# UniBwTAS/continuous_clustering

Measured on AMD Instinct MI355X. Metric: Mpoints/s clustered (64-beam streams), higher is better.
Workload: dtype f32

## Files before the change

continuous_clustering_amd/csrc/cc_device.h:

```cpp
#pragma once
#include <stdint.h>
#include <hip/hip_runtime.h>

#include "../../include/cc_hip.h"

namespace ccd
{

constexpr int WAVE = 64;
constexpr int MAX_ROWS_PER_LANE = 2;
constexpr int LINK_SLOTS = 4;
constexpr int WIN_COLS = 32;
constexpr int PP_SKIP = 0x7fffffff;
#ifndef CC_INS_WIN
#define CC_INS_WIN 64
#endif
constexpr int INS_WIN = CC_INS_WIN;
constexpr int SG_NAN = 1, SG_FOG = 2, SG_EGO = 4, SG_INCL_IGNORE = 8, SG_TOO_CLOSE = 16, SG_PENDING = 32;
constexpr unsigned NAN_RANGE_BITS = 0x7fc00001u;
#ifndef CC_TREE_SLOTS
#define CC_TREE_SLOTS 256
#endif
constexpr int TREE_SLOTS = CC_TREE_SLOTS;
#ifndef CC_TABLE_WAVES
// ... 47 lines not shown
    uint64_t exceed_one_rotation;
    uint64_t serial_columns;
    uint64_t stamp_alias_rounds;
    uint64_t batch_columns;
    uint64_t batch_bails;
    uint64_t batch_bail_reason[8];
    int64_t par_clear_done;
    int32_t par_bad;
    int32_t par_upto;
    int64_t serial_until;
    uint64_t dbg[16];
    int32_t error;
    int32_t n_events;
    int64_t error_a;
    int64_t error_b;
    int32_t n_links;
    int32_t pad2;
    int64_t overrun_col;
};

struct Planes
{
    float* dist;
    float* incl;
    float* incaz;
    uint16_t* gtag;
    uint32_t* src;
    uint8_t* inten;
    int32_t* trig;
    int64_t* colg;
    double* colminaz;
    uint8_t* ground;
    uint8_t* debug;
    uint8_t* ignored;
    int32_t* root;
    uint32_t* id;
    double* t_fin;
    uint32_t* t_width;
    uint32_t* t_pts;
    int32_t* t_uf;
    uint32_t* t_cid;
    int32_t* t_pos;
    uint8_t* t_finished;
    int32_t* ulist;
    int32_t* ucomp;
    unsigned long long* agg_fin;
    long long* agg_min;
// ... 65 lines not shown
```

continuous_clustering_amd/csrc/cc_engine.hip:

```cpp
#include <hip/hip_runtime.h>

#include <algorithm>
#include <chrono>
#include <cstdlib>
#include <cmath>
#include <cstdio>
#include <cstring>
#include <functional>
#include <limits>
#include <mutex>
#include <string>
#include <vector>

#include "cc_kernels.h"

#ifndef CC_LWAVE_MAX_STREAMS
#define CC_LWAVE_MAX_STREAMS 256
#endif

using namespace ccd;

struct cc_engine
{
    int device{0};
// ... 277 lines not shown
    e->d_small_seq = nullptr;
    e->d_input_sum = nullptr;
    e->small_view_ok = false;
    e->small_seq_expected = 0;
    free_pinned(e, PIN_SHAPE);
    return CC_OK;
}

int allocate(cc_engine* e)
{
    const Geometry& g = e->g;
    const size_t S = (size_t) g.num_streams;
    const size_t C = S * (size_t) g.cells;
    const size_t L = S * (size_t) g.ring_cols;
    const size_t T = S * (size_t) g.tree_capacity;
    Planes& P = e->P;
    int rc = CC_OK;
    e->slab_planning = getenv("CC_NO_SLAB") == nullptr;
    e->slab_bytes = 0;
    e->slab_plan.clear();
#define A(field, count)                                \
    if ((rc = alloc_plane(e, &P.field, (count))) != 0) \
        return rc;
    A(dist, C) A(incl, C) A(incaz, C) A(gtag, C) A(src, C) A(inten, C);
    A(trig, L) A(colg, L) A(colminaz, L);
    A(ground, C) A(debug, C) A(ignored, C) A(root, C) A(id, C);
    A(t_fin, C) A(t_width, C) A(t_pts, C) A(t_uf, C) A(t_cid, C) A(t_pos, C) A(t_finished, C);
    A(ulist, T) A(ucomp, T) A(agg_fin, T) A(agg_min, T) A(agg_max, T) A(agg_pts, T) A(agg_cid, T) A(agg_first, T) A(agg_flag, T);
    A(events, S * (size_t) g.event_capacity);
    A(sc_parent, C) A(sc_nlinks, C) A(sc_links, C) A(sc_fin, C);
    A(sc_term, C) A(col_newfin, L) A(col_info, L) A(col_act, L) A(pk_meta, C) A(pk_fin, C) A(pk_lk, C);
    A(sg_x2, C) A(sg_uz, C) A(sg_w, C) A(sg_flags, C) A(sc_rec, C);
    A(curtab, S * (size_t) g.num_rows);
    A(tab_acc, S * (size_t) g.tab_tiles * (size_t) g.num_rows);
    A(par_off, S * (size_t) cck::IP_MAXF);
    A(tabc, (size_t) BATCH_SLOTS * S * (size_t) g.tab_tiles * (size_t) g.num_rows);
    A(sc_visits, C);
    A(link_log, S * (size_t) g.link_capacity);
    A(sl_ctl, S * 4) A(sl_cols, L);
    if ((rc = alloc_plane(e, (unsigned long long**) &P.sl_rec, S * (size_t) cck::SL_CAP * sizeof(cck::ScanLongRec) / sizeof(unsigned long long))) != 0)
        return rc;
#undef A
    if ((rc = alloc_plane(e, &e->d_states, S)) != 0)
        return rc;
    if ((rc = alloc_plane(e, &e->d_par_left, 16)) != 0)
        return rc;
    if ((rc = alloc_plane(e, &e->d_bail_count, 4)) != 0)
// ... 31 lines not shown
    st.clear_done = -1;
    st.first_unpublished = -1;
    st.cluster_counter = 1;
    st.min_required = 0;
    st.finish_lower_bound = std::numeric_limits<double>::max();
    st.last_round_min_az = -1.0;
    st.overrun_col = std::numeric_limits<int64_t>::max();
    st.n_links = 0;
    for (auto& d : st.batch)
        d.seg_begin = d.seg_end = d.acp_next = d.pub_begin = d.pub_end = -1, d.mode = 0, d.fused = 0;
    st.assoc_mode = e->cfg.max_steps_in_row > WIN_COLS - 2 ? 1 : 0;
}

int reset_state(cc_engine* e, bool keep_table)
{
    e->small_view_ok = false;
    e->widest_steps_in_row = e->cfg.max_steps_in_row;
    std::fill(e->state_cached.begin(), e->state_cached.end(), 0);
    const Geometry& g = e->g;
    const size_t S = (size_t) g.num_streams;
    const size_t C = S * (size_t) g.cells;
    Planes& P = e->P;
    CC_HIP_CHECK(e, hipMemsetAsync(P.dist, 0xFF, C * sizeof(float), e->stream));
    CC_HIP_CHECK(e, hipMemsetAsync(P.incl, 0xFF, C * sizeof(float), e->stream));
    CC_HIP_CHECK(e, hipMemsetAsync(P.gtag, 0, C * sizeof(uint16_t), e->stream));
    CC_HIP_CHECK(e, hipMemsetAsync(P.id, 0, C * sizeof(uint32_t), e->stream));
    CC_HIP_CHECK(e, hipMemsetAsync(P.ground, CC_GP_UNKNOWN, C, e->stream));
    CC_HIP_CHECK(e, hipMemsetAsync(P.debug, CC_DBG_WHITE, C, e->stream));
    CC_HIP_CHECK(e, hipMemsetAsync(P.ignored, 0, C, e->stream));
    CC_HIP_CHECK(e, hipMemsetAsync(P.root, 0xFF, C * sizeof(int32_t), e->stream));
    CC_HIP_CHECK(e, hipMemsetAsync(P.tab_acc, 0, S * (size_t) g.tab_tiles * (size_t) g.num_rows * sizeof(unsigned long long), e->stream));
    CC_HIP_CHECK(e, hipMemsetAsync(P.sl_ctl, 0, S * 4 * sizeof(int32_t), e->stream));
    if (!keep_table)
        CC_HIP_CHECK(e, hipMemsetAsync(P.curtab, 0xFF, S * (size_t) g.num_rows * sizeof(float), e->stream));
    std::vector<StreamState> init(S);
    for (auto& st : init)
        fresh_stream_state(e, &st);
    CC_HIP_CHECK(e, hipMemcpyAsync(e->d_states, init.data(), S * sizeof(StreamState), hipMemcpyHostToDevice, e->stream));
    if (e->d_take_cursor)
        CC_HIP_CHECK(e, hipMemsetAsync(e->d_take_cursor, 0, 2 * S * sizeof(long long), e->stream));
    if (e->d_tc_cursor)
        CC_HIP_CHECK(e, hipMemsetAsync(e->d_tc_cursor, 0, 2 * S * sizeof(long long), e->stream));
    CC_HIP_CHECK(e, hipStreamSynchronize(e->stream));
    for (auto& v : e->pending_events)
        v.clear();
    for (auto& v : e->pending_links)
        v.clear();
    e->batch_open = false;
    for (bool& b : e->assoc_pending)
        b = false;
    e->deferred_tail = nullptr;
    e->lazy_pending = false;
    e->lazy_prev_left = nullptr;
    e->lazy_miss = 0;
    e->lazy_clean = 0;
    e->lazy_ok = true;
    return CC_OK;
}

int reset_streams_state(cc_engine* e, const std::vector<int>& list)
{
    const Geometry& g = e->g;
    const Planes& P = e->P;
    const unsigned long long cells = (unsigned long long) g.cells;
    cck::ResetJob job;
    memset(&job, 0, sizeof(job));
    const cck::ResetFill fills[cck::RESET_PLANES] = {
        {(char*) P.dist, cells * sizeof(float), 0xFF, 0},
        {(char*) P.incl, cells * sizeof(float), 0xFF, 0},
        {(char*) P.gtag, cells * sizeof(uint16_t), 0, 0},
        {(char*) P.id, cells * sizeof(uint32_t), 0, 0},
        {(char*) P.ground, cells, CC_GP_UNKNOWN, 0},
        {(char*) P.debug, cells, CC_DBG_WHITE, 0},
        {(char*) P.ignored, cells, 0, 0},
        {(char*) P.root, cells * sizeof(int32_t), 0xFF, 0},
        {(char*) P.tab_acc, (unsigned long long) g.tab_tiles * (unsigned long long) g.num_rows * sizeof(unsigned long long), 0, 0},
        {(char*) P.sl_ctl, 4 * sizeof(int32_t), 0, 0},
    };
    unsigned long long longest = 0;
    for (int k = 0; k < cck::RESET_PLANES; k++)
    {
        job.fill[k] = fills[k];
        longest = std::max(longest, fills[k].bytes);
    }
    fresh_stream_state(e, &job.fresh);
    job.states = e->d_states;
    job.take_cursor = e->d_take_cursor;
    job.tc_cursor = e->d_tc_cursor;
    job.num_streams = g.num_streams;
    int rc = ensure_gather(e, list.size() * sizeof(int));
    if (rc)
        return rc;
// ... 527 lines not shown
    const int64_t RC = e->g.ring_cols;
    const size_t off = (size_t) stream * (size_t) e->g.cells + (size_t) (st.overrun_col % RC) * R;
    if (hipMemcpy(col.data(), e->P.gtag + off, (size_t) R * sizeof(uint16_t), hipMemcpyDeviceToHost) != hipSuccess)
        return;
    const unsigned tag = 0x8000u | ((unsigned) (st.overrun_col / RC) & 0x7fffu);
    for (int row = R - 1; row >= 0; row--)
        if (col[(size_t) row] != tag && col[(size_t) row] != 0)
        {
            st.error_a = st.overrun_col - (int64_t) ((tag - (unsigned) col[(size_t) row]) & 0x7fffu) * RC;
            st.error_b = st.overrun_col;
            return;
        }
}

void restore_table_after_overrun(cc_engine* e, int stream, const StreamState& st)
{
    if (st.error != CC_ERR_RING_OVERRUN || st.overrun_col == std::numeric_limits<int64_t>::max())
        return;
    const int R = e->g.num_rows;
    const int64_t RC = e->g.ring_cols, c = st.overrun_col;
    const int64_t oldest = std::max<int64_t>(0, c - (RC - 2 * (int64_t) e->g.num_columns));
    const size_t base = (size_t) stream * (size_t) e->g.cells;
    float* curtab = e->P.curtab + (size_t) stream * (size_t) R;
    std::vector<float> table((size_t) R), incl, dist;
    std::vector<uint16_t> tags;
    std::vector<uint8_t> found((size_t) R, 0);
    if (hipMemcpy(table.data(), curtab, (size_t) R * sizeof(float), hipMemcpyDeviceToHost) != hipSuccess)
        return;
    int missing = R;
    for (int64_t hi = c - 1; hi >= oldest && missing > 0;)
    {
        const int64_t lo = std::max(std::max(oldest, hi - 255), hi - hi % RC);
        const size_t n = (size_t) (hi - lo + 1) * (size_t) R, off = base + (size_t) (lo % RC) * (size_t) R;
        incl.resize(n), dist.resize(n), tags.resize(n);
        if (hipMemcpy(incl.data(), e->P.incl + off, n * sizeof(float), hipMemcpyDeviceToHost) != hipSuccess ||
            hipMemcpy(dist.data(), e->P.dist + off, n * sizeof(float), hipMemcpyDeviceToHost) != hipSuccess ||
            hipMemcpy(tags.data(), e->P.gtag + off, n * sizeof(uint16_t), hipMemcpyDeviceToHost) != hipSuccess)
            return;
        for (int64_t g = hi; g >= lo && missing > 0; g--)
        {
            const unsigned tag = 0x8000u | ((unsigned) (g / RC) & 0x7fffu);
            const size_t o = (size_t) (g - lo) * (size_t) R;
            float below = 0.f;
            for (int row = R - 1; row >= 0; row--)
            {
                const bool has = tags[o + (size_t) row] == tag && !std::isnan(dist[o + (size_t) row]);
                const float cur = has ? incl[o + (size_t) row] : std::nanf("");
                const float diff = cur - below;
                if (!std::isnan(diff) && !found[(size_t) row])
                {
                    table[(size_t) row] = diff;
                    found[(size_t) row] = 1;
                    missing--;
                }
                below = cur;
            }
        }
        hi = lo - 1;
    }
    (void) hipMemcpy(curtab, table.data(), (size_t) R * sizeof(float), hipMemcpyHostToDevice);
}

void set_kernel_error(cc_engine* e, int stream, StreamState& st)
{
    fixup_overrun(e, stream, st);
    restore_table_after_overrun(e, stream, st);
    char buf[320];
    if (st.error == CC_ERR_RING_OVERRUN)
        snprintf(buf, sizeof(buf), "stream %d: This column is not cleared (ring buffer full or written after clearing): %lld, %lld, %d", stream,
                 (long long) st.error_a, (long long) st.error_b, e->g.ring_cols);
// ... 1711 lines not shown
```

continuous_clustering_amd/csrc/cc_k_base.h:

```cpp
#pragma once

#define CC_PI_F 3.14159274101257324219f
#define CC_2PI_D 6.283185307179586

__device__ __forceinline__ int lane_id()
{
    return threadIdx.x & 63;
}

__device__ __forceinline__ int f2i_x86(float v)
{
    if (!(v > -2147483904.0f && v < 2147483648.0f))
        return (int) 0x80000000;
    return (int) v;
}

template<int CTRL, int ROW_MASK>
__device__ __forceinline__ int dpp_mov_i32(int fill, int v)
{
    return __builtin_amdgcn_update_dpp(fill, v, CTRL, ROW_MASK, 0xf, false);
}
template<int CTRL, int ROW_MASK>
__device__ __forceinline__ long long dpp_mov_i64(long long fill, long long v)
{
// ... 210 lines not shown
    }
    return m;
}
__device__ __forceinline__ void caz_key(const float packed, int& kpos, int& kneg)
{
    const unsigned u = __float_as_uint(packed);
    const int k = (int) (u & 0x7fffffffu);
    if (u >> 31)
        kneg = k < kneg ? k : kneg;
    else
        kpos = k < kpos ? k : kpos;
}

constexpr uint16_t CELL_CLEARED = 0;
__device__ __forceinline__ uint16_t cell_tag(const long long pass)
{
    return (uint16_t) (0x8000u | ((unsigned) pass & 0x7fffu));
}

constexpr int IP_MAXF = 4608;

struct SP
{
    float *dist, *incl, *tabc;
    float* incaz;
    uint16_t* gtag;
    uint32_t* src;
    uint8_t *inten, *ground, *debug, *ignored;
    int32_t* trig;
    int64_t* colg;
    double* colminaz;
    int32_t* root;
    uint32_t* id;
    double* t_fin;
    uint32_t *t_width, *t_pts, *t_cid;
    int32_t *t_uf, *t_pos;
    uint8_t* t_finished;
    int32_t *ulist, *ucomp;
    unsigned long long* agg_fin;
    long long *agg_min, *agg_max;
    uint32_t *agg_pts, *agg_cid;
    int32_t* agg_first;
    uint8_t* agg_flag;
    float* curtab;
    unsigned long long* tab_acc;
    int32_t* par_off;
    cc_event* events;
// ... 3 lines not shown
    int32_t* col_info;
    uint16_t* col_act;
    unsigned* pk_meta;
    double* pk_fin;
    unsigned long long* pk_lk;
    uint8_t* sc_nlinks;
    unsigned long long* sc_links;
    double* sc_fin;
    float *sg_x2, *sg_uz, *sg_w;
    uint8_t* sg_flags;
    float4* sc_rec;
    uint16_t* sc_visits;
    int2* link_log;
    int32_t* sl_cols;
};

__device__ __forceinline__ SP stream_ptrs(const Planes& P, const Geometry& g, int s)
{
    SP p;
    const size_t co = (size_t) s * (size_t) g.cells;
    const size_t lo = (size_t) s * (size_t) g.ring_cols;
    const size_t to = (size_t) s * (size_t) g.tree_capacity;
    p.dist = P.dist + co;
    p.incl = P.incl + co;
    p.incaz = P.incaz + co;
    p.gtag = P.gtag + co;
    p.src = P.src + co;
    p.inten = P.inten + co;
    p.ground = P.ground + co;
    p.debug = P.debug + co;
    p.ignored = P.ignored + co;
    p.trig = P.trig + lo;
    p.colg = P.colg + lo;
    p.colminaz = P.colminaz + lo;
    p.root = P.root + co;
    p.id = P.id + co;
    p.t_fin = P.t_fin + co;
    p.t_width = P.t_width + co;
    p.t_pts = P.t_pts + co;
    p.t_cid = P.t_cid + co;
    p.t_uf = P.t_uf + co;
    p.t_pos = P.t_pos + co;
    p.t_finished = P.t_finished + co;
    p.ulist = P.ulist + to;
    p.ucomp = P.ucomp + to;
    p.agg_fin = P.agg_fin + to;
    p.agg_min = P.agg_min + to;
// ... 44 lines not shown
```

continuous_clustering_amd/csrc/cc_k_insert.h:

```cpp
#pragma once

struct PreppedPoint
{
    float x, y, z, dist, incl, incaz;
    int cir;
};

__device__ __forceinline__ PreppedPoint prep_point(const float fx, const float fy, const float fz, const double* __restrict__ T, const bool clockwise,
                                                   const float az_width)
{
    PreppedPoint o;
    o.x = o.y = o.z = o.dist = o.incl = o.incaz = 0.f;
    o.cir = PP_SKIP;
    if (fx != fx)
        return o;
    const double px = fx, py = fy, pz = fz;
    const double tx = T[3], ty = T[7], tz = T[11];
    const double ox = ((T[0] * px + T[1] * py) + T[2] * pz) + tx;
    const double oy = ((T[4] * px + T[5] * py) + T[6] * pz) + ty;
    const double oz = ((T[8] * px + T[9] * py) + T[10] * pz) + tz;
    const double rx = ox - tx, ry = oy - ty, rz = oz - tz;
    const float az = ccm::atan2f_exact(fy, fx);
    const float inc_az = clockwise ? -az + CC_PI_F : az + CC_PI_F;
    const float dist = (float) __builtin_sqrt((rx * rx + ry * ry) + rz * rz);
// ... 176 lines not shown
    if (st->pre_seg_begin > 0)
    {
        seg_begin = st->pre_seg_begin;
        limit_base = st->pre_seg_begin;
    }
    unsigned long long negative_cols = 0;
    bool ring_init = false;

    long long clear_done = st->clear_done;
    if (clear_done >= 0)
    {
        const long long clear_to = ring_start < st->clear_allowed ? ring_start : st->clear_allowed;
        for (; clear_done < clear_to; clear_done++)
        {
            const int clc = (int) (clear_done % RC);
#pragma unroll
            for (int k = 0; k < RPL; k++)
            {
                const int row = k * 64 + lane;
                if (row < R)
                {
                    const size_t ci = (size_t) clc * R + row;
                    p.dist[ci] = __builtin_nanf("");
                    p.incl[ci] = __builtin_nanf("");
                    p.gtag[ci] = CELL_CLEARED;
                }
            }
        }
    }

    long long wbase = -1;
    auto window_fill = [&](long long from, long long to)
    {
        int lcx = (int) (from % RC);
        constexpr int B = 16;
        for (long long g0 = from; g0 < to; g0 += B)
        {
            float v[B][RPL];
            int lcs = lcx;
#pragma unroll
            for (int u = 0; u < B; u++)
            {
#pragma unroll
                for (int k = 0; k < RPL; k++)
                {
                    const int row = k * 64 + lane;
                    v[u][k] = 0.f;
// ... 141 lines not shown
                {
                    lc += RC;
                    pass--;
                }
                else if (lc >= RC)
                {
                    lc -= RC;
                    pass++;
                }
                const uint16_t tag0 = cell_tag(pass);
#pragma unroll
                for (int k = 0; k < RPL; k++)
                {
                    const int row = k * 64 + lane;
                    if (v[k])
                    {
                        const int so = slot * R + row;
                        const size_t ci = (size_t) lc * R + row;
                        const float d = r_d[so];
                        p.sc_rec[ci] = make_float4(r_x[so], r_y[so], r_z[so], r_i[so]);
                        p.inten[ci] = (uint8_t) r_t[so];
                        p.src[ci] = (uint32_t) (seq0 + (f - cursor0));
                        p.dist[ci] = d;
                        p.incl[ci] = r_i[so];
                        p.incaz[ci] = pack_incaz(r_a[so], c0 >= NC);
                        p.gtag[ci] = tag0;
                        w_dist[wcol + row] = d;
                    }
                }
                if (gc0 > prev_rear)
                {
                    const int dlt = (int) (gc0 - prev_rear);
                    prev_rear = gc0;
                    prev_cir += dlt;
                    if (prev_cir >= NC)
                    {
                        prev_cir -= NC;
                        prev_rot++;
                    }
                    rear_lc += dlt;
                    if (rear_lc >= RC)
                    {
                        rear_lc -= RC;
                        rear_pass++;
                    }
                    tracked_rear = prev_rear;
                }
// ... 168 lines not shown
                    float nd = lds_ld(&w_dist[res ? (int) ((gc + 1) & (WINC - 1)) * R + row : row]);
                    if (__any(!res))
                    {
                        if (!res)
                            nd = ld_agent(&p.dist[(size_t) (lc + 1 >= RC ? 0 : lc + 1) * R + row]);
                    }
                    if (nd != nd)
                    {
                        gc++;
                        pass += lc + 1 >= RC ? 1 : 0;
                        lc = lc + 1 >= RC ? 0 : lc + 1;
                        cd = nd;
                    }
                }
                if (!(cd != cd) && ((d != d) || d >= cd))
                    continue;
                const bool too_far_behind = first_unf >= 0 && gc < first_unf;
                if (!too_far_behind)
                {
                    const size_t ci = (size_t) lc * R + row;
                    p.sc_rec[ci] = make_float4(r_x[so], r_y[so], r_z[so], r_i[so]);
                    p.inten[ci] = (uint8_t) r_t[so];
                    p.src[ci] = (uint32_t) (seq0 + (f - cursor0));
                    p.incl[ci] = r_i[so];
                    p.incaz[ci] = pack_incaz(r_a[so], cir[k] + (int) (gc - gcv[k]) >= NC);
                    p.gtag[ci] = cell_tag(pass);
                    p.dist[ci] = d;
                    if (!NOWIN && gc >= wbase && gc < wbase + WINC)
                        w_dist[(int) (gc & (WINC - 1)) * R + row] = d;
                }
                l_rear = gc < l_rear ? gc : l_rear;
                l_fore = gc > l_fore ? gc : l_fore;
            }
#ifdef CC_PROFILE_SECTIONS
            CC_ISEC(2)
#endif
            {
                const int span = (int) (need_hi + 1 - need_lo);
                int o_lo = l_fore >= 0 ? (int) (l_rear - need_lo) : 0x7fffffff;
                int o_hi = l_fore >= 0 ? (int) (l_fore - need_lo) : -1;
                if (span <= 1)
                {
                    const unsigned long long lo0 = __ballot(o_lo == 0), hi1 = __ballot(o_hi == 1), any = __ballot(o_hi >= 0);
                    if (any)
                    {
                        rear = need_lo + (lo0 ? 0 : 1);
                        fore = need_lo + (hi1 ? 1 : 0);
// ... 122 lines not shown

template<int RPL>
__global__ __launch_bounds__(128) void k_insert2(Geometry g, cc_config cfg, Planes P, StreamState* states, int first_stream, int slot,
                                                 const uint8_t* __restrict__ inten, long long n, int* remaining, long long n_total, long long fbase)
{
    insert2_body<RPL>(g, cfg, P, states, first_stream, slot, inten, n, remaining, n_total, fbase, (int) blockIdx.x);
}

template<int RPL>
__device__ __forceinline__ void par_take_back(const SP& p, const int R, const int RC, const int lc0, const int rel_from, const int rel_to, const int wave,
                                              const int nwaves, const int lane)
{
    for (int rel = rel_from + wave; rel <= rel_to; rel += nwaves)
    {
        const int lc = (int) ((unsigned) (lc0 + rel) % (unsigned) RC);
#pragma unroll
        for (int k = 0; k < RPL; k++)
        {
            const int row = k * 64 + lane;
            if (row < R)
            {
                const size_t ci = (size_t) lc * R + row;
                p.dist[ci] = __builtin_nanf("");
                p.incl[ci] = __builtin_nanf("");
                p.gtag[ci] = CELL_CLEARED;
            }
        }
    }
}

__device__ __forceinline__ int par_close_stream(StreamState* st, const int slot, int* left_over, const bool fuse, const bool whole, const int done,
                                                const long long n, const long long prev_rear0, const long long first_unf0, const long long ring_end0,
                                                const long long seq0, const long long rel_last)
{
    (void) n;
    int fused = 0;
    if (done > 0)
    {
        const long long G = prev_rear0 + rel_last;
        st->prev_rearmost = G;
        st->prev_foremost = G;
        st->first_unfinished = G;
        if (G > ring_end0)
            st->ring_end = G;
        st->cursor = done;
        st->firings_consumed = (unsigned long long) (seq0 + done);
        st->pre_seg_begin = first_unf0;
// ... 275 lines not shown
        {
            __shared__ long long s_clear_to;
            if (tid == 0)
            {
                const long long want = clear_to > clear_done ? clear_to : clear_done;
                const unsigned long long seen = atomicCAS((unsigned long long*) &st->par_clear_done, ~0ull, (unsigned long long) want);
                s_clear_to = seen == ~0ull ? want : (long long) seen;
            }
            __syncthreads();
            clear_to = s_clear_to;
        }
        const int cstep = W * nby;
        int clc = (int) ((clear_done + wave + W * by) % RC);
        for (long long c = clear_done + wave + W * by; c < clear_to; c += cstep, clc = clc + cstep >= RC ? clc + cstep - RC : clc + cstep)
        {
#pragma unroll
            for (int k = 0; k < RPL; k++)
            {
                const int row = k * 64 + lane;
                if (row < R)
                {
                    const size_t ci = (size_t) clc * R + row;
                    p.dist[ci] = __builtin_nanf("");
                    p.incl[ci] = __builtin_nanf("");
                    p.gtag[ci] = CELL_CLEARED;
                }
            }
        }
        if (clear_to > clear_done)
            clear_done = clear_to;
    }
    const bool steady = st->cursor == 0 && ring_start != -1 && first_unf0 > 0 && first_unf0 == prev_rear0 && prev_fore0 == prev_rear0 &&
                        st->reset_required == 0 && st->pre_seg_begin == 0 && clear_done >= 0;
    const int nn = (int) (n < IP_MAXF ? n : IP_MAXF);
    if (tid == 0)
    {
        s_upto = nn;
        s_carry = 0;
    }
    __syncthreads();
    if (!steady)
    {
        if (tid == 0 && by == 0)
        {
            if (nby == 1)
                st->clear_done = clear_done;
            if (left_over)
// ... 348 lines not shown
        const long long rel_prev = f > 0 ? s_off[f - 1] : 0;
        const long long G = prev_rear0 + rel;
        int lc;
        const int lcq = div_small(lc0 + (int) rel, RC, rcp_rc, lc);
        const uint16_t tag = cell_tag(pass0 + (long long) lcq);
        const bool seg_here = fuse && f + 1 < upto;
#pragma unroll
        for (int k = 0; k < RPL; k++)
        {
            const int row = k * 64 + lane;
            const unsigned ci = (unsigned) lc * (unsigned) R + (unsigned) row;
            const bool has = q[k].cir != PP_SKIP;
            if (has | (seg_here & (row < R)))
            {
                const float nn = __builtin_nanf("");
                at32(p.sc_rec, ci) = make_float4(has ? q[k].x : nn, has ? q[k].y : nn, has ? q[k].z : nn, has ? q[k].incl : nn);
                at32(p.gtag, ci) = tag;
            }
            if (has)
            {
                at32(p.inten, ci) = cint[k];
                at32(p.src, ci) = (uint32_t) (seq0 + f);
                at32(p.dist, ci) = q[k].dist;
                at32(p.incl, ci) = q[k].incl;
                at32(p.incaz, ci) = q[k].incaz;
            }
        }
        const int cnt = (int) (rel - rel_prev);
        for (int jj = lane; jj < cnt; jj += 64)
        {
            int tlc;
            (void) div_small(lc0 + (int) rel_prev + jj, RC, rcp_rc, tlc);
            p.trig[tlc] = f;
        }
        if (seg_here)
        {
            float sx[RPL], sy[RPL], sz[RPL], sd[RPL], si_[RPL], saz[RPL], x2[RPL], uz[RPL], w[RPL];
            int flags[RPL];
#pragma unroll
            for (int k = 0; k < RPL; k++)
            {
                const bool has = q[k].cir != PP_SKIP;
                sx[k] = q[k].x, sy[k] = q[k].y, sz[k] = q[k].z, saz[k] = q[k].incaz;
                sd[k] = has ? q[k].dist : __builtin_nanf("");
                si_[k] = has ? q[k].incl : __builtin_nanf("");
            }
            const double* E = ego + ((size_t) sl * (size_t) n + (size_t) (uniform_i32(f) + 1)) * EGO_STRIDE;
// ... 135 lines not shown
    }
    const long long prev_rear0 = uniform_i64(st->prev_rearmost), prev_fore0 = uniform_i64(st->prev_foremost), first_unf0 = uniform_i64(st->first_unfinished);
    const long long ring_end0 = uniform_i64(st->ring_end);
    if (tid == 0)
        s_ring_start = __hip_atomic_load(&st->ring_start, __ATOMIC_RELAXED, __HIP_MEMORY_SCOPE_AGENT);
    __syncthreads();
    const long long ring_start = uniform_i64(s_ring_start);
    long long clear_done = uniform_i64(st->clear_done);
    if (clear_done >= 0)
    {
        const long long clear_allowed = uniform_i64(st->clear_allowed);
        const long long clear_to = ring_start < clear_allowed ? ring_start : clear_allowed;
        for (long long c = clear_done + wave; c < clear_to; c += IM_WAVES)
        {
            const int clc = (int) (c % RC);
#pragma unroll
            for (int k = 0; k < RPL; k++)
            {
                const int row = k * 64 + lane;
                if (row < R)
                {
                    const size_t ci = (size_t) clc * R + row;
                    p.dist[ci] = __builtin_nanf("");
                    p.incl[ci] = __builtin_nanf("");
                    p.gtag[ci] = CELL_CLEARED;
                }
            }
        }
        if (clear_to > clear_done)
            clear_done = clear_to;
    }
    const bool steady = ring_start != -1 && first_unf0 > 0 && first_unf0 == prev_rear0 && prev_fore0 >= prev_rear0 && st->reset_required == 0 &&
                        clear_done >= 0 && prev_fore0 - prev_rear0 < NC / 2;
    __syncthreads();
    if (!steady)
    {
        if (tid == 0)
        {
            st->clear_done = clear_done;
            if (left_over)
                atomicAdd(left_over, 1);
        }
        return;
    }
    for (int r = tid; r < NR; r += 64 * IM_WAVES)
        s_rowmax[r] = (int) 0x80000000;
#if CC_IM_STAGE
// ... 269 lines not shown
            if (__any(clash) && lane == 0)
                atomicMin(&s_stop, wave);
        }
        IM_MARK(2)
        lds_barrier();
        IM_MARK(3)
        {
            const int st2 = uniform_i32(s_stop);
            stop = st2 < stop ? st2 : stop;
        }
        if (mine && wave < stop)
        {
#pragma unroll
            for (int k = 0; k < RPL; k++)
            {
                const int row = k * 64 + lane;
                if (oc[k] >= 0)
                {
                    const int crel = my_rel + oc[k];
                    const unsigned lcq = (unsigned) (lc0 + crel) / (unsigned) RC;
                    const int lc = (int) ((unsigned) (lc0 + crel) - lcq * (unsigned) RC);
                    const unsigned ci = (unsigned) lc * (unsigned) R + (unsigned) row;
                    at32(p.sc_rec, ci) = make_float4(q[k].x, q[k].y, q[k].z, q[k].incl);
                    at32(p.incl, ci) = q[k].incl;
#if !CC_IM_STAGE
                    at32(p.inten, ci) = cint[k];
                    at32(p.src, ci) = (uint32_t) (seq0 + (f - cursor0));
                    at32(p.dist, ci) = q[k].dist;
                    at32(p.incaz, ci) = q[k].incaz;
                    at32(p.gtag, ci) = cell_tag(pass0 + (long long) lcq);
#else
                    int slot = base_slot + (crel - base_rel);
                    slot = slot >= IM_W ? slot - IM_W : slot;
#if CC_IM_STAGE_DIST
                    s_dist[slot][row] = q[k].dist;
#else
                    at32(p.dist, ci) = q[k].dist;
#endif
                    s_int[slot][row] = cint[k];
                    s_fw[slot][row] = (unsigned char) (0x80u | ((unsigned) (f - cursor0) & 127u));
#if CC_IM_STAGE_INCAZ
                    s_incaz[slot][row] = q[k].incaz;
#else
                    at32(p.incaz, ci) = q[k].incaz;
#endif
#endif
                    atomicMax(&s_rowmax[row], crel);
// ... 78 lines not shown
```

continuous_clustering_amd/csrc/cc_k_publish.h:

```cpp
#pragma once

constexpr int PUBLISH_BLOCKS = 64;

struct ViewOut
{
    float *x, *y, *z, *dist, *incl;
    double* caz;
    int64_t *gcol, *src, *root_gcol;
    uint8_t *ground, *debug, *ignored;
    uint64_t* id;
    int32_t* root_row;
    double* fin;
    uint32_t *tpts, *width, *nchild;
    int32_t *visits, *par_row;
    uint8_t* finished;
    int64_t* par_gcol;
};


__device__ __forceinline__ void view_column(const Geometry& g, const SP& p, const StreamState* st, const long long gc, const int oc, const ViewOut& o)
{
    const int R = g.num_rows, RC = g.ring_cols;
    const int lc = (int) (((gc % RC) + RC) % RC);
    const bool in_ring = st->ring_end >= 0 && gc >= 0 && gc >= st->clear_done && gc <= st->ring_end;
    const bool segmented = in_ring && st->first_column >= 0 && gc >= st->first_column && gc < st->first_unfinished;
    const CazBase cb = caz_base_of_column(gc >= 0 ? gc : 0, g.num_columns);
    const uint16_t tag = cell_tag((gc >= 0 ? gc : 0) / RC);
    for (int row = lane_id(); row < R; row += 64)
    {
        const size_t ci = (size_t) lc * R + row;
        const size_t oi = (size_t) oc * R + row;
        const float nanf_ = __builtin_nanf("");
        const bool mine = p.gtag[ci] == tag;
        const bool filled = in_ring && (segmented ? true : mine);
        const bool has_point = filled && !(p.dist[ci] != p.dist[ci]) && mine;
        const bool has_record = has_point || (filled && mine && __float_as_uint(p.dist[ci]) == NAN_RANGE_BITS);
        const float4 rec = has_record ? p.sc_rec[ci] : make_float4(nanf_, nanf_, nanf_, nanf_);
        o.x[oi] = rec.x;
        o.y[oi] = rec.y;
        o.z[oi] = rec.z;
        o.dist[oi] = has_point ? p.dist[ci] : nanf_;
        o.incl[oi] = (has_point || segmented) ? p.incl[ci] : nanf_;
        o.caz[oi] = has_point ? cell_caz(cb, p.incaz[ci]) : (segmented ? empty_cell_caz(gc, g.az_width) : __builtin_nan(""));
        o.gcol[oi] = segmented ? gc : (has_point ? gc : -1);
        o.src[oi] = has_record ? (long long) (st->firings_consumed - (unsigned long long) (uint32_t) ((uint32_t) st->firings_consumed - p.src[ci])) : -1;
        o.ground[oi] = segmented ? p.ground[ci] : (uint8_t) CC_GP_UNKNOWN;
        o.debug[oi] = segmented ? p.debug[ci] : (uint8_t) CC_DBG_WHITE;
        o.ignored[oi] = segmented ? p.ignored[ci] : 0;
        const int r = segmented ? p.root[ci] : -1;
        o.id[oi] = r >= 0 ? (uint64_t) p.t_cid[r] : 0ull;
        o.root_gcol[oi] = r >= 0 ? p.colg[r / R] : -1;
        o.root_row[oi] = r >= 0 ? r % R : 0;
        const bool is_root = r >= 0 && (size_t) r == ci;
        if (o.fin)
            o.fin[oi] = is_root ? p.t_fin[ci] : 0.;
        if (o.tpts)
            o.tpts[oi] = is_root ? p.t_pts[ci] : 0u;
        if (o.width)
            o.width[oi] = is_root ? p.t_width[ci] : 0u;
        if (o.finished)
            o.finished[oi] = is_root ? p.t_finished[ci] : (uint8_t) 0;
        if (o.visits)
            o.visits[oi] = (segmented && g.mirror_fields) ? (int32_t) p.sc_visits[ci] : 0;
        const int code = (segmented && r >= 0) ? (int) p.sc_parent[ci] : -1;
        if (o.par_gcol)
// ... 563 lines not shown
```

continuous_clustering_amd/csrc/cc_k_reset.h:

```cpp
#pragma once

constexpr int RESET_PLANES = 10;
constexpr int RESET_THREADS = 256;
constexpr unsigned long long RESET_CHUNK_BYTES = 16384;
constexpr int RESET_MAX_BLOCKS = 2048;
static_assert(sizeof(StreamState) % sizeof(unsigned long long) == 0 && alignof(StreamState) == alignof(unsigned long long), "the state is copied in 8-byte words");

struct ResetFill
{
    char* plane;
    unsigned long long bytes;
    unsigned value;
    unsigned pad;
};

struct ResetJob
{
    ResetFill fill[RESET_PLANES];
    StreamState fresh;
    StreamState* states;
    long long* take_cursor;
    long long* tc_cursor;
    int num_streams;
    int pad;
};
// ... 40 lines not shown
```

continuous_clustering_amd/csrc/cc_k_segment.h:

```cpp
#pragma once


template<int RPL>
__device__ __forceinline__ void table_scan_tiles(const SP& p, const int R, const int ntiles, const int lane)
{
    float carry[RPL];
#pragma unroll
    for (int k = 0; k < RPL; k++)
    {
        const int row = k * 64 + lane;
        carry[k] = row < R ? p.curtab[row] : 0.f;
    }
    constexpr int U = 8;
    for (int t0 = 0; t0 < ntiles; t0 += U)
    {
        float v[U][RPL];
#pragma unroll
        for (int u = 0; u < U; u++)
#pragma unroll
            for (int k = 0; k < RPL; k++)
            {
                const int row = k * 64 + lane;
                v[u][k] = (row < R && t0 + u < ntiles) ? p.tabc[(size_t) (t0 + u) * R + row] : __builtin_nanf("");
            }
// ... 24 lines not shown
__global__ __launch_bounds__(64 * TABLE_WAVES) void k_table(Geometry g, Planes P, StreamState* states, int first_stream, int slot)
{
    const int s = first_stream + blockIdx.x;
    const int lane = lane_id(), wave = uniform_i32((int) (threadIdx.x >> 6));
    StreamState* st = &states[s];
#ifdef CC_CHAIN2_PRIO
    __builtin_amdgcn_s_setprio(CC_CHAIN2_PRIO);
#endif
    if (threadIdx.x == 0)
        st->batch[slot].mode = st->assoc_mode;
    const long long seg_begin = st->batch[slot].seg_begin, seg_end = st->batch[slot].seg_end;
    if (seg_begin < 0 || seg_begin >= seg_end)
        return;
    if (st->batch[slot].fused)
        return;
    const SP p = stream_ptrs(P, g, s);
    const int R = g.num_rows, RC = g.ring_cols;
    const int ntiles = (int) ((seg_end - seg_begin + 63) >> 6);
    constexpr int U = 16;
    for (int t = wave; t < ntiles; t += TABLE_WAVES)
    {
        const long long c_lo = seg_begin + 64ll * t, c_hi = (c_lo + 64 < seg_end ? c_lo + 64 : seg_end);
        float last[RPL];
#pragma unroll
        for (int k = 0; k < RPL; k++)
            last[k] = __builtin_nanf("");
        int lc = (int) (c_lo % RC);
        for (long long c0 = c_lo; c0 < c_hi; c0 += U)
        {
            float cur[U][RPL], below[U][RPL];
#pragma unroll
            for (int u = 0; u < U; u++)
            {
#pragma unroll
                for (int k = 0; k < RPL; k++)
                {
                    const int row = k * 64 + lane;
                    cur[u][k] = below[u][k] = 0.f;
                    if (row < R && c0 + u < c_hi)
                    {
                        const size_t ci = (size_t) lc * R + row;
                        cur[u][k] = p.incl[ci];
                        below[u][k] = row + 1 < R ? p.incl[ci + 1] : 0.f;
                    }
                }
                lc = lc + 1 == RC ? 0 : lc + 1;
            }
#pragma unroll
            for (int u = 0; u < U; u++)
            {
                if (c0 + u >= c_hi)
                    break;
#pragma unroll
                for (int k = 0; k < RPL; k++)
                {
                    const float diff = cur[u][k] - below[u][k];
                    if (!(diff != diff))
                        last[k] = diff;
                }
            }
        }
#pragma unroll
        for (int k = 0; k < RPL; k++)
        {
            const int row = k * 64 + lane;
            if (row < R)
                p.tabc[(size_t) t * R + row] = last[k];
        }
    }
    __syncthreads();
    if (wave == 0)
        table_scan_tiles<RPL>(p, R, ntiles, lane);
}

__device__ __forceinline__ void ego_record(const StreamState* __restrict__ states, int first_stream, const cc_config& cfg, const double* __restrict__ poses,
                                           long long n, long long n_total, long long fbase, double* __restrict__ out, const int sl, const long long f)
{
    const double* A = states[first_stream + sl].robot_from_sensor;
    const double* T = poses + ((size_t) sl * (size_t) n_total + (size_t) fbase + (size_t) f) * 12;
    double ir[9], it[3];
    for (int i = 0; i < 3; i++)
        for (int j = 0; j < 3; j++)
            ir[i * 3 + j] = T[j * 4 + i];
// ... 183 lines not shown
        if (__any(overrun))
        {
            const int worst = -wave_min_i32(-overrun_row);
            if (overrun_row == worst)
            {
                atomicMin((unsigned long long*) &st->overrun_col, (unsigned long long) gc);
                raise_error(st, CC_ERR_RING_OVERRUN, overrun_gcol, gc);
            }
            continue;
        }
        float x2[RPL], uz[RPL], w[RPL];
        int flags[RPL];
        seg_pre_cells<RPL>(cfg, R, lane, cx, cy, cz, dist, incl, n_inten, spx, spy, spz, E, x2, uz, w, flags);
        int kpos = 0x7fffffff, kneg = 0x7fffffff;
        bool any_empty = false;
#pragma unroll
        for (int k = 0; k < RPL; k++)
        {
            const int row = k * 64 + lane;
            if (row >= R)
                continue;
            const size_t ci = base + row;
            if (empty_cell[k])
                p.gtag[ci] = tag;
            if (flags[k] & SG_NAN)
                any_empty = true;
            else
                caz_key(n_incaz[k], kpos, kneg);
            p.sg_x2[ci] = x2[k];
            p.sg_uz[ci] = uz[k];
            p.sg_w[ci] = w[k];
            p.sg_flags[ci] = (uint8_t) flags[k];
        }
        const double min_az = column_min_caz(cb, kpos, kneg, any_empty, gc, g.az_width);
        if (lane == 0)
        {
            p.colg[lc] = gc;
            p.colminaz[lc] = min_az;
        }
    }
}

#ifndef CC_SEGSCAN_MIN_WAVES_PER_SIMD
#define CC_SEGSCAN_MIN_WAVES_PER_SIMD 2
#endif
constexpr int SEG_X2_RING = 16;
constexpr int SEG_CH = 16;
// ... 35 lines not shown
    if (tile0 >= seg_end)
        return;
    const int ncols = (int) (seg_end - tile0 < 64 ? seg_end - tile0 : 64);
    const SP p = stream_ptrs(P, g, s);
    const int R = g.num_rows, RC = g.ring_cols;
    const int lane = lane_id();
    const int PF = seg_pitch_f(R), PB = seg_pitch_b(R);
    const bool tiled = seg_tiled(R);
    extern __shared__ __attribute__((aligned(16))) unsigned char smem[];
    float* l_x2 = (float*) smem;
    unsigned char* l_out = (unsigned char*) (l_x2 + (tiled ? 4 * 64 * SEG_CH : 64 * PF));

    const int lc0 = (int) (tile0 % RC);
    {
        const bool active = lane < ncols;
        const long long gc = tile0 + lane;
        int lcl = lc0 + lane;
        lcl = lcl >= RC ? lcl - RC : lcl;
        const float* gx = p.sg_x2 + (size_t) lcl * R;
        const float* gz = p.sg_uz + (size_t) lcl * R;
        const float* gw = p.sg_w + (size_t) lcl * R;
        const unsigned char* gf = p.sg_flags + (size_t) lcl * R;
        float4* g_rec = p.sc_rec + (size_t) lcl * R;
        float* g_incl = p.incl + (size_t) lcl * R;
        const float* tab_in = p.tabc + (size_t) blockIdx.y * R;
        unsigned char* oo = l_out + lane * PB;
        const float height_sensor_to_ground = -(float) st->robot_from_sensor[11] + cfg.height_ref_to_ground_;
        const bool chess_odd = cfg.ignore_points_in_chessboard_pattern && (gc & 1);
        const bool chess_even = cfg.ignore_points_in_chessboard_pattern && !(gc & 1);
        bool first_obstacle_detected = false, first_point_found = false;
        float lg2x = 0.f, lgz = height_sensor_to_ground;
        float pv2x = 0.f, pvz = 0.f;
        unsigned char previous_label = 0;
        auto row_step = [&](const int row, const int f, const float cur2x, const float cur2y, auto&& x2_below)
        {
            const bool valid = (f & (SG_NAN | SG_FOG | SG_EGO)) == 0;
            const bool first = valid & !first_point_found;
            const bool normal = valid & first_point_found;
            const bool ign = ((f & (SG_TOO_CLOSE | SG_INCL_IGNORE)) != 0) | ((row & 1) ? chess_even : chess_odd);
            const float h = cur2y - height_sensor_to_ground;
            const bool first_ground = (h > cfg.first_ring_as_ground_min_allowed_z_diff) & (h < cfg.first_ring_as_ground_max_allowed_z_diff);
            const float p2cx = cur2x - pv2x, p2cy = cur2y - pvz;
            const float slope_to_prev = p2cy / p2cx;
            const bool flat_prev = (ccm::absf(slope_to_prev) < cfg.max_slope) & (p2cx > 0) & ((cfg.use_terrain == 0) | (p2cx < 5));
            const float l2cx = cur2x - lg2x, l2cy = cur2y - lgz;
            const float slope_to_lg = l2cy / l2cx;
            const bool flat_lg = (ccm::absf(slope_to_lg) < cfg.max_slope) & (l2cx > 0);
// ... 43 lines not shown
            lgz = new_lg ? cur2y : lgz;
            pv2x = valid ? cur2x : pv2x;
            pvz = valid ? cur2y : pvz;
            previous_label = valid ? (unsigned char) d : previous_label;
            first_point_found |= valid;
            oo[row] = (unsigned char) (g | (d << 3) | ((valid & ign) ? 0x80u : 0u));
        };
        const unsigned long long le_mask = lane == 63 ? ~0ull : ((2ull << lane) - 1ull);
        const bool supplement = cfg.supplement_inclination_angle_for_nan_cells != 0;
        const bool step_filter = cfg.ignore_points_with_too_big_inclination_angle_diff != 0;
        float supp_below = __builtin_nanf("");
        bool below_nan = false;
        auto row_all = [&](const int row, const int f, const float cur2x, const float cur2y, const float wv, const float carry, auto&& x2_below,
                           auto&& stash) -> bool
        {
            const bool own = !(f & (SG_NAN | SG_PENDING));
            const unsigned long long m = __ballot(own) & le_mask;
            const int src = m ? 63 - __clzll((long long) m) : lane;
            const float got = __shfl(wv, src, 64);
            const float tab = m ? got : carry;
            const bool is_nan = (f & SG_NAN) != 0;
            const float supp = (supplement & (row < R - 1)) ? (below_nan ? supp_below : wv) + tab : __builtin_nanf("");
            if (is_nan & active)
            {
                g_rec[row].w = supp;
                g_incl[row] = supp;
            }
            supp_below = is_nan ? supp : supp_below;
            below_nan = is_nan;
            const bool pend = ((f & (SG_PENDING | SG_NAN)) == SG_PENDING) & step_filter & (row < R - 1) & !(tab != tab);
            const float a = wv * tab;
            const bool in_range = (cfg.max_distance > 0.f) & (tab >= 0.f) & (tab < 0.05f) & (wv > 0.f) & (wv < 3.0e38f);
            const bool surely_not = in_range & (cfg.max_distance >= 1.01f * a);
            const bool surely = in_range & !surely_not & (cfg.max_distance * 1.000002f < a);
            const int fx = f | ((pend & surely) ? SG_INCL_IGNORE : 0);
            const bool need = pend & !surely_not & !surely;
            if (need)
                stash(tab);
            row_step(row, fx, cur2x, cur2y, x2_below);
            return need;
        };
        if (tiled && ncols <= SEG_FEW && 3 * SEG_FEW * R <= 4 * 64 * SEG_CH)
        {
            float* cx2 = l_x2;
            float* cuz = l_x2 + SEG_FEW * R;
            float* cw = l_x2 + 2 * SEG_FEW * R;
            for (int c = 0; c < ncols; c++)
            {
                int l = lc0 + c;
                l = l >= RC ? l - RC : l;
// ... 458 lines not shown
            const bool reached = has_ra & ((NP & le & ~le_ra) == 0);
            if (reached & (gl == (unsigned) SG_G_GROUND))
            {
                gl = SG_G_OBSTACLE;
                d = SG_D_DARKRED;
            }
        }
        if (inrow)
        {
            constexpr unsigned long long GV = (unsigned long long) CC_GP_UNKNOWN | ((unsigned long long) CC_GP_GROUND << 8) |
                                              ((unsigned long long) CC_GP_OBSTACLE << 16) | ((unsigned long long) CC_GP_EGO_VEHICLE << 24) |
                                              ((unsigned long long) CC_GP_FOG << 32);
            constexpr unsigned long long DV0 = (unsigned long long) CC_DBG_WHITE | ((unsigned long long) CC_DBG_GRAY << 8) |
                                               ((unsigned long long) CC_DBG_ORANGE << 16) | ((unsigned long long) CC_DBG_GREEN << 24) |
                                               ((unsigned long long) CC_DBG_YELLOWGREEN << 32) | ((unsigned long long) CC_DBG_YELLOW << 40) |
                                               ((unsigned long long) CC_DBG_RED << 48) | ((unsigned long long) CC_DBG_DARKRED << 56);
            constexpr unsigned DV1 = (unsigned) CC_DBG_VIOLET | ((unsigned) CC_DBG_LIGHTGRAY << 8);
            p.ground[ci] = (unsigned char) (GV >> (8 * gl));
            p.debug[ci] = (unsigned char) (d < 8 ? (DV0 >> (8 * d)) : (unsigned long long) (DV1 >> (8 * (d - 8))));
            p.ignored[ci] = (gl != (unsigned) SG_G_OBSTACLE || ign) ? 1 : 0;
            if (empty_cell)
                p.gtag[ci] = tag;
            if (is_nan)
            {
                p.sc_rec[ci].w = sincl;
                p.incl[ci] = sincl;
            }
        }
        int kpos = 0x7fffffff, kneg = 0x7fffffff;
        if (inrow && !is_nan)
            caz_key(incaz, kpos, kneg);
        const double min_az = column_min_caz(cb, kpos, kneg, inrow && is_nan, gc, g.az_width);
        if (lane == 0)
        {
            p.colg[lc] = gc;
            p.colminaz[lc] = min_az;
        }
        lc = lc + 1 == RC ? 0 : lc + 1;
        pass += lc == 0 ? 1 : 0;
        cir = cir + 1 == NC ? 0 : cir + 1;
        if (cir == 0)
        {
            rot++;
            cb = caz_base_of_rotation(rot);
        }
    }
    if (inrow)
        p.curtab[row] = tabrow;
}

// ... 7 lines not shown
```

Before: 19840.

## Drop duplicate incl plane and read inclination from sc_rec.w with backward scan

```diff
diff --git a/continuous_clustering_amd/csrc/cc_device.h b/continuous_clustering_amd/csrc/cc_device.h
--- a/continuous_clustering_amd/csrc/cc_device.h
+++ b/continuous_clustering_amd/csrc/cc_device.h
@@ -93,7 +93,6 @@
 struct Planes
 {
     float* dist;
-    float* incl;
     float* incaz;
     uint16_t* gtag;
     uint32_t* src;
diff --git a/continuous_clustering_amd/csrc/cc_engine.hip b/continuous_clustering_amd/csrc/cc_engine.hip
--- a/continuous_clustering_amd/csrc/cc_engine.hip
+++ b/continuous_clustering_amd/csrc/cc_engine.hip
@@ -323,7 +323,7 @@
 #define A(field, count)                                \
     if ((rc = alloc_plane(e, &P.field, (count))) != 0) \
         return rc;
-    A(dist, C) A(incl, C) A(incaz, C) A(gtag, C) A(src, C) A(inten, C);
+    A(dist, C) A(incaz, C) A(gtag, C) A(src, C) A(inten, C);
     A(trig, L) A(colg, L) A(colminaz, L);
     A(ground, C) A(debug, C) A(ignored, C) A(root, C) A(id, C);
     A(t_fin, C) A(t_width, C) A(t_pts, C) A(t_uf, C) A(t_cid, C) A(t_pos, C) A(t_finished, C);
@@ -401,7 +401,6 @@
     const size_t C = S * (size_t) g.cells;
     Planes& P = e->P;
     CC_HIP_CHECK(e, hipMemsetAsync(P.dist, 0xFF, C * sizeof(float), e->stream));
-    CC_HIP_CHECK(e, hipMemsetAsync(P.incl, 0xFF, C * sizeof(float), e->stream));
     CC_HIP_CHECK(e, hipMemsetAsync(P.gtag, 0, C * sizeof(uint16_t), e->stream));
     CC_HIP_CHECK(e, hipMemsetAsync(P.id, 0, C * sizeof(uint32_t), e->stream));
     CC_HIP_CHECK(e, hipMemsetAsync(P.ground, CC_GP_UNKNOWN, C, e->stream));
@@ -446,7 +445,6 @@
     memset(&job, 0, sizeof(job));
     const cck::ResetFill fills[cck::RESET_PLANES] = {
         {(char*) P.dist, cells * sizeof(float), 0xFF, 0},
-        {(char*) P.incl, cells * sizeof(float), 0xFF, 0},
         {(char*) P.gtag, cells * sizeof(uint16_t), 0, 0},
         {(char*) P.id, cells * sizeof(uint32_t), 0, 0},
         {(char*) P.ground, cells, CC_GP_UNKNOWN, 0},
@@ -1020,7 +1018,8 @@
     const int64_t oldest = std::max<int64_t>(0, c - (RC - 2 * (int64_t) e->g.num_columns));
     const size_t base = (size_t) stream * (size_t) e->g.cells;
     float* curtab = e->P.curtab + (size_t) stream * (size_t) R;
-    std::vector<float> table((size_t) R), incl, dist;
+    std::vector<float> table((size_t) R), dist;
+    std::vector<float4> rec;
     std::vector<uint16_t> tags;
     std::vector<uint8_t> found((size_t) R, 0);
     if (hipMemcpy(table.data(), curtab, (size_t) R * sizeof(float), hipMemcpyDeviceToHost) != hipSuccess)
@@ -1030,8 +1029,8 @@
     {
         const int64_t lo = std::max(std::max(oldest, hi - 255), hi - hi % RC);
         const size_t n = (size_t) (hi - lo + 1) * (size_t) R, off = base + (size_t) (lo % RC) * (size_t) R;
-        incl.resize(n), dist.resize(n), tags.resize(n);
-        if (hipMemcpy(incl.data(), e->P.incl + off, n * sizeof(float), hipMemcpyDeviceToHost) != hipSuccess ||
+        rec.resize(n), dist.resize(n), tags.resize(n);
+        if (hipMemcpy(rec.data(), e->P.sc_rec + off, n * sizeof(float4), hipMemcpyDeviceToHost) != hipSuccess ||
             hipMemcpy(dist.data(), e->P.dist + off, n * sizeof(float), hipMemcpyDeviceToHost) != hipSuccess ||
             hipMemcpy(tags.data(), e->P.gtag + off, n * sizeof(uint16_t), hipMemcpyDeviceToHost) != hipSuccess)
             return;
@@ -1043,7 +1042,7 @@
             for (int row = R - 1; row >= 0; row--)
             {
                 const bool has = tags[o + (size_t) row] == tag && !std::isnan(dist[o + (size_t) row]);
-                const float cur = has ? incl[o + (size_t) row] : std::nanf("");
+                const float cur = has ? rec[o + (size_t) row].w : std::nanf("");
                 const float diff = cur - below;
                 if (!std::isnan(diff) && !found[(size_t) row])
                 {
diff --git a/continuous_clustering_amd/csrc/cc_k_base.h b/continuous_clustering_amd/csrc/cc_k_base.h
--- a/continuous_clustering_amd/csrc/cc_k_base.h
+++ b/continuous_clustering_amd/csrc/cc_k_base.h
@@ -256,7 +256,7 @@
 
 struct SP
 {
-    float *dist, *incl, *tabc;
+    float *dist, *tabc;
     float* incaz;
     uint16_t* gtag;
     uint32_t* src;
@@ -306,7 +306,6 @@
     const size_t lo = (size_t) s * (size_t) g.ring_cols;
     const size_t to = (size_t) s * (size_t) g.tree_capacity;
     p.dist = P.dist + co;
-    p.incl = P.incl + co;
     p.incaz = P.incaz + co;
     p.gtag = P.gtag + co;
     p.src = P.src + co;
diff --git a/continuous_clustering_amd/csrc/cc_k_insert.h b/continuous_clustering_amd/csrc/cc_k_insert.h
--- a/continuous_clustering_amd/csrc/cc_k_insert.h
+++ b/continuous_clustering_amd/csrc/cc_k_insert.h
@@ -222,7 +222,6 @@
                 {
                     const size_t ci = (size_t) clc * R + row;
                     p.dist[ci] = __builtin_nanf("");
-                    p.incl[ci] = __builtin_nanf("");
                     p.gtag[ci] = CELL_CLEARED;
                 }
             }
@@ -410,7 +409,6 @@
                         p.inten[ci] = (uint8_t) r_t[so];
                         p.src[ci] = (uint32_t) (seq0 + (f - cursor0));
                         p.dist[ci] = d;
-                        p.incl[ci] = r_i[so];
                         p.incaz[ci] = pack_incaz(r_a[so], c0 >= NC);
                         p.gtag[ci] = tag0;
                         w_dist[wcol + row] = d;
@@ -625,7 +623,6 @@
                     p.sc_rec[ci] = make_float4(r_x[so], r_y[so], r_z[so], r_i[so]);
                     p.inten[ci] = (uint8_t) r_t[so];
                     p.src[ci] = (uint32_t) (seq0 + (f - cursor0));
-                    p.incl[ci] = r_i[so];
                     p.incaz[ci] = pack_incaz(r_a[so], cir[k] + (int) (gc - gcv[k]) >= NC);
                     p.gtag[ci] = cell_tag(pass);
                     p.dist[ci] = d;
@@ -794,7 +791,6 @@
             {
                 const size_t ci = (size_t) lc * R + row;
                 p.dist[ci] = __builtin_nanf("");
-                p.incl[ci] = __builtin_nanf("");
                 p.gtag[ci] = CELL_CLEARED;
             }
         }
@@ -1116,7 +1112,6 @@
                 {
                     const size_t ci = (size_t) clc * R + row;
                     p.dist[ci] = __builtin_nanf("");
-                    p.incl[ci] = __builtin_nanf("");
                     p.gtag[ci] = CELL_CLEARED;
                 }
             }
@@ -1511,7 +1506,6 @@
                 at32(p.inten, ci) = cint[k];
                 at32(p.src, ci) = (uint32_t) (seq0 + f);
                 at32(p.dist, ci) = q[k].dist;
-                at32(p.incl, ci) = q[k].incl;
                 at32(p.incaz, ci) = q[k].incaz;
             }
         }
@@ -1693,7 +1687,6 @@
                 {
                     const size_t ci = (size_t) clc * R + row;
                     p.dist[ci] = __builtin_nanf("");
-                    p.incl[ci] = __builtin_nanf("");
                     p.gtag[ci] = CELL_CLEARED;
                 }
             }
@@ -2009,7 +2002,6 @@
                     const int lc = (int) ((unsigned) (lc0 + crel) - lcq * (unsigned) RC);
                     const unsigned ci = (unsigned) lc * (unsigned) R + (unsigned) row;
                     at32(p.sc_rec, ci) = make_float4(q[k].x, q[k].y, q[k].z, q[k].incl);
-                    at32(p.incl, ci) = q[k].incl;
 #if !CC_IM_STAGE
                     at32(p.inten, ci) = cint[k];
                     at32(p.src, ci) = (uint32_t) (seq0 + (f - cursor0));
diff --git a/continuous_clustering_amd/csrc/cc_k_publish.h b/continuous_clustering_amd/csrc/cc_k_publish.h
--- a/continuous_clustering_amd/csrc/cc_k_publish.h
+++ b/continuous_clustering_amd/csrc/cc_k_publish.h
@@ -31,16 +31,18 @@
         const size_t ci = (size_t) lc * R + row;
         const size_t oi = (size_t) oc * R + row;
         const float nanf_ = __builtin_nanf("");
-        const bool mine = p.gtag[ci] == tag;
+        const uint16_t tg = p.gtag[ci];
+        const bool mine = tg == tag;
         const bool filled = in_ring && (segmented ? true : mine);
         const bool has_point = filled && !(p.dist[ci] != p.dist[ci]) && mine;
         const bool has_record = has_point || (filled && mine && __float_as_uint(p.dist[ci]) == NAN_RANGE_BITS);
-        const float4 rec = has_record ? p.sc_rec[ci] : make_float4(nanf_, nanf_, nanf_, nanf_);
-        o.x[oi] = rec.x;
-        o.y[oi] = rec.y;
-        o.z[oi] = rec.z;
+        const bool has_incl = has_point || (segmented && tg != CELL_CLEARED);
+        const float4 rec = (has_record || has_incl) ? p.sc_rec[ci] : make_float4(nanf_, nanf_, nanf_, nanf_);
+        o.x[oi] = has_record ? rec.x : nanf_;
+        o.y[oi] = has_record ? rec.y : nanf_;
+        o.z[oi] = has_record ? rec.z : nanf_;
         o.dist[oi] = has_point ? p.dist[ci] : nanf_;
-        o.incl[oi] = (has_point || segmented) ? p.incl[ci] : nanf_;
+        o.incl[oi] = has_incl ? rec.w : nanf_;
         o.caz[oi] = has_point ? cell_caz(cb, p.incaz[ci]) : (segmented ? empty_cell_caz(gc, g.az_width) : __builtin_nan(""));
         o.gcol[oi] = segmented ? gc : (has_point ? gc : -1);
         o.src[oi] = has_record ? (long long) (st->firings_consumed - (unsigned long long) (uint32_t) ((uint32_t) st->firings_consumed - p.src[ci])) : -1;
diff --git a/continuous_clustering_amd/csrc/cc_k_reset.h b/continuous_clustering_amd/csrc/cc_k_reset.h
--- a/continuous_clustering_amd/csrc/cc_k_reset.h
+++ b/continuous_clustering_amd/csrc/cc_k_reset.h
@@ -1,6 +1,6 @@
 #pragma once
 
-constexpr int RESET_PLANES = 10;
+constexpr int RESET_PLANES = 9;
 constexpr int RESET_THREADS = 256;
 constexpr unsigned long long RESET_CHUNK_BYTES = 16384;
 constexpr int RESET_MAX_BLOCKS = 2048;
diff --git a/continuous_clustering_amd/csrc/cc_k_segment.h b/continuous_clustering_amd/csrc/cc_k_segment.h
--- a/continuous_clustering_amd/csrc/cc_k_segment.h
+++ b/continuous_clustering_amd/csrc/cc_k_segment.h
@@ -70,43 +70,80 @@
     {
         const long long c_lo = seg_begin + 64ll * t, c_hi = (c_lo + 64 < seg_end ? c_lo + 64 : seg_end);
         float last[RPL];
+        bool found[RPL];
 #pragma unroll
         for (int k = 0; k < RPL; k++)
+        {
             last[k] = __builtin_nanf("");
-        int lc = (int) (c_lo % RC);
-        for (long long c0 = c_lo; c0 < c_hi; c0 += U)
-        {
-            float cur[U][RPL], below[U][RPL];
+            found[k] = k * 64 + lane >= R;
+        }
+        int lc = (int) ((c_hi - 1) % RC);
+        long long pass = (c_hi - 1) / RC;
+        for (long long c0 = c_hi - 1; c0 >= c_lo; c0 -= U)
+        {
+            uint16_t tcur[U][RPL], tbel[U][RPL];
+            int lcs[U];
+            uint16_t tags[U];
+            {
+                int l = lc;
+                long long ps = pass;
+#pragma unroll
+                for (int u = 0; u < U; u++)
+                {
+                    lcs[u] = l;
+                    tags[u] = cell_tag(ps);
+#pragma unroll
+                    for (int k = 0; k < RPL; k++)
+                    {
+                        const int row = k * 64 + lane;
+                        tcur[u][k] = tbel[u][k] = CELL_CLEARED;
+                        if (row < R && c0 - u >= c_lo)
+                        {
+                            const size_t ci = (size_t) l * R + row;
+                            tcur[u][k] = p.gtag[ci];
+                            tbel[u][k] = row + 1 < R ? p.gtag[ci + 1] : tags[u];
+                        }
+                    }
+                    ps -= l == 0 ? 1 : 0;
+                    l = l == 0 ? RC - 1 : l - 1;
+                }
+                lc = l;
+                pass = ps;
+            }
+            bool all_found = true;
 #pragma unroll
             for (int u = 0; u < U; u++)
             {
+                bool cand[RPL], any = false;
 #pragma unroll
                 for (int k = 0; k < RPL; k++)
                 {
+                    cand[k] = !found[k] && tcur[u][k] == tags[u] && tbel[u][k] == tags[u];
+                    any |= cand[k];
+                }
+                if (!__any(any))
+                    continue;
+#pragma unroll
+                for (int k = 0; k < RPL; k++)
+                {
                     const int row = k * 64 + lane;
-                    cur[u][k] = below[u][k] = 0.f;
-                    if (row < R && c0 + u < c_hi)
+                    if (cand[k])
                     {
-                        const size_t ci = (size_t) lc * R + row;
-                        cur[u][k] = p.incl[ci];
-                        below[u][k] = row + 1 < R ? p.incl[ci + 1] : 0.f;
+                        const size_t ci = (size_t) lcs[u] * R + row;
+                        const float diff = p.sc_rec[ci].w - (row + 1 < R ? p.sc_rec[ci + 1].w : 0.f);
+                        if (!(diff != diff))
+                        {
+                            last[k] = diff;
+                            found[k] = true;
+                        }
                     }
                 }
-                lc = lc + 1 == RC ? 0 : lc + 1;
-            }
-#pragma unroll
-            for (int u = 0; u < U; u++)
-            {
-                if (c0 + u >= c_hi)
-                    break;
-#pragma unroll
-                for (int k = 0; k < RPL; k++)
-                {
-                    const float diff = cur[u][k] - below[u][k];
-                    if (!(diff != diff))
-                        last[k] = diff;
-                }
-            }
+            }
+#pragma unroll
+            for (int k = 0; k < RPL; k++)
+                all_found &= found[k];
+            if (__all(all_found))
+                break;
         }
 #pragma unroll
         for (int k = 0; k < RPL; k++)
@@ -336,7 +373,10 @@
                 continue;
             const size_t ci = base + row;
             if (empty_cell[k])
+            {
                 p.gtag[ci] = tag;
+                p.sc_rec[ci].w = __builtin_nanf("");
+            }
             if (flags[k] & SG_NAN)
                 any_empty = true;
             else
@@ -418,7 +458,6 @@
         const float* gw = p.sg_w + (size_t) lcl * R;
         const unsigned char* gf = p.sg_flags + (size_t) lcl * R;
         float4* g_rec = p.sc_rec + (size_t) lcl * R;
-        float* g_incl = p.incl + (size_t) lcl * R;
         const float* tab_in = p.tabc + (size_t) blockIdx.y * R;
         unsigned char* oo = l_out + lane * PB;
         const float height_sensor_to_ground = -(float) st->robot_from_sensor[11] + cfg.height_ref_to_ground_;
@@ -508,10 +547,7 @@
             const bool is_nan = (f & SG_NAN) != 0;
             const float supp = (supplement & (row < R - 1)) ? (below_nan ? supp_below : wv) + tab : __builtin_nanf("");
             if (is_nan & active)
-            {
                 g_rec[row].w = supp;
-                g_incl[row] = supp;
-            }
             supp_below = is_nan ? supp : supp_below;
             below_nan = is_nan;
             const bool pend = ((f & (SG_PENDING | SG_NAN)) == SG_PENDING) & step_filter & (row < R - 1) & !(tab != tab);
@@ -1016,10 +1052,7 @@
             if (empty_cell)
                 p.gtag[ci] = tag;
             if (is_nan)
-            {
                 p.sc_rec[ci].w = sincl;
-                p.incl[ci] = sincl;
-            }
         }
         int kpos = 0x7fffffff, kneg = 0x7fffffff;
         if (inrow && !is_nan)
```

Result: no change. 19730 (-0.5%).
